# ELEKTRONN/ELEKTRONN2

Measured on AMD Instinct MI355X. Metric: training_input_voxels_per_sec, higher is better.
Workload: dtype f32; 1 GPU; neuro3d_lite (1,1,23,183,183)->(1,2,10,37,37) fwd+bwd+Adam, 1 sample/GPU; parallelism=dp1, hipgraph=True, steps_per_launch=10

## Files before the change

### elektronn2_amd/autotune.py

```python
from __future__ import annotations

import json
import math
import os

from .backend import E2Error

_HERE = os.path.dirname(os.path.abspath(__file__))
_SHIPPED = os.path.join(_HERE, "tuned.json")
_cache = None
_dirty = False
IGEMM_MTS = [1, 2, 3, 4, 5, 6, 7, 8, 10, 13]
WGRAD_MTS = [1, 2, 3, 4, 5, 7]


def _cache_path():
    return os.environ.get("E2HIP_TUNE_CACHE", os.path.join(_HERE, ".tune_cache.json"))


def _load():
    global _cache
    if _cache is None:
        _cache = {}
        for path in (_SHIPPED, _cache_path()):
# ... 101 lines not shown


def g4_pairs(mg, nt, kw):
    na = (4 * mg + 63) // 64
    u = 1
    while u < 8 and u * kw * mg * nt < 40 and 2 * (2 * u) * kw * (na + nt) + 4 * mg * nt <= 88:
        u *= 2
    return u


def igemm4_candidates(cout, cin, k, out_sp, split_k=True, n_cu=256):
    if k[2] not in (1, 3, 4, 5):
        return []
    q = out_sp[1] * out_sp[2]
    cinp = -(-cin // 4) * 4
    groups = -(-cout // 4)
    shapes = []
    for mg, nt in IGEMM4_INSTANCES:
        for wm in range(1, 13):
            bm = 4 * mg * wm
            nmt = -(-cout // bm)
            pad = nmt * bm - cout
            if pad >= 4 * mg and wm > 1:
                continue
            if nmt > 1 and wm < 3 and mg * wm < groups / 4.0:
                continue
            for wn in (1, 2, 3, 4, 6, 12):
                if wm * wn > 12 or (wm * wn < 6 and wm * wn != 4):
                    continue
                shapes.append((round(pad / float(cout), 3), -wm * wn, mg, nt, wm, wn, nmt))
    shapes.sort()
    best_pad = shapes[0][0] if shapes else 0
    cands = []
    for padf, _, mg, nt, wm, wn, nmt in shapes:
        if padf > best_pad + 0.06:
            break
        u = g4_pairs(mg, nt, k[2])
        step = u * 4 // math.gcd(u, 4)
        if ((step // u) * k[1]) % 2:
            step *= 2
        bn = 64 * nt * wn
        if bn > 2 * q:
            continue
        base = out_sp[0] * (-(-q // bn)) * nmt
        sks = (1,) if (base >= 160 or not split_k) else (1, 2, 4)
        ccs = sorted(set(-(-c // step) * step for c in (8, 16) if c >= 4))
        ccs = [c for c in ccs if -(-cin // c) * c <= cinp + 32][:2]
        for cc in ccs:
            for sk in sks:
                tiles = base * sk
                for g in (1, 2):
                    if g > 1 and (tiles <= n_cu or wm * wn > 6):
                        continue
                    cands.append("4,%d,%d,%d,%d,%d,%d,%d" % (mg, nt, cc, sk, wm, wn, g))
    return cands


def wgrad_candidates(cout, cin, k, out_sp, n_cu=256):
    mblocks = -(-cout // 16)
    T = k[0] * k[1] * k[2]
    nblocks = -(-(cin * T) // 16)
    q = out_sp[1] * out_sp[2]
    qpad = out_sp[1] * (out_sp[2] + 2 * (k[2] - 1))
    cands = []
    for mt in _best_mts(mblocks, WGRAD_MTS, keep=3):
        nmt = -(-mblocks // mt)
        variants = [(1, 1), (2, 1), (4, 1), (2, 14), (4, 14), (1, 0), (2, 0), (4, 0)]
        if nblocks <= 2:
            variants = [(1, 4), (1, 0), (1, 1), (2, 14)]
        for nt, wk in variants:
            wn = 1 if wk in (4, 14) else 4
            if nt > 1 and 16 * nt * wn > 16 * nblocks:
                continue
            nnt = -(-nblocks // (nt * wn))
            for bp in ((128, 256) if wk in (1, 14) else (64, 128)):
                tiles = out_sp[0] * (-(-(qpad if wk in (1, 14) else q) // bp))
                for fill in (1, 1.5, 2, 3, 4):
                    ps = max(1, min(tiles, int(n_cu * fill) // max(1, nmt * nnt)))
                    for q in {ps} | set(_near_divisors(tiles, ps)):
                        cands.append("%d,%d,%d,%d,%d" % (mt, nt, wk, bp, q))
                        if wk in (1, 14) and nnt >= 2 and nmt * q * nnt > 8:
                            cands.append("%d,%d,%d,%d,%d" % (mt, nt, wk + 100, bp, q))
    return sorted(set(cands) | set(pointwise_wgrad_candidates(cout, cin, k, out_sp, n_cu))
                  | set(position_split_wgrad_candidates(cout, cin, k, out_sp, n_cu)))


WGRAD_KS_TILES = [(13, 2), (10, 2), (8, 2), (8, 4), (7, 2), (7, 4), (6, 4), (5, 4), (4, 4), (3, 4), (2, 4)]


def position_split_wgrad_candidates(cout, cin, k, out_sp, n_cu=256):
    T = k[0] * k[1] * k[2]
    if T == 1 or cout < 24:
        return []
    pitch = out_sp[2] + k[2] - 1
    if (k[1] - 1) * pitch + k[2] - 1 < 31:
        return []
    units = out_sp[0] * (-(-((out_sp[1] - 1) * pitch + out_sp[2]) // 32))
    scored = []
    for mt, nt in WGRAD_KS_TILES:
        nm, nn = -(-cout // (16 * mt)), -(-(cin * T) // (16 * nt))
        eff = (cout * cin * T) / float(nm * 16 * mt * nn * 16 * nt)
        scored.append((-eff, -mt * nt, mt, nt, nm * nn))
    scored.sort()
    out = []
    for _, _, mt, nt, tiles in scored[:4]:
        for fill in (0.5, 1, 2):
            s = max(1, min(-(-units // 4), int(n_cu * fill) // tiles))
            out.append("%d,%d,9,0,%d" % (mt, nt, s))
    return sorted(set(out))


PW_WGRAD_KS_TILES = [(13, 2), (10, 2), (7, 2), (7, 4), (4, 4)]
PW_WGRAD_TILES = [(2, 2), (4, 2), (2, 4), (4, 4), (4, 3), (3, 4), (7, 2), (2, 7), (7, 4), (4, 7)]


def pointwise_wgrad_candidates(cout, cin, k, out_sp, n_cu=256):
    if tuple(k) != (1, 1, 1) or cout < 32 or cin < 32:
        return []
    steps = -(-(out_sp[0] * out_sp[1] * out_sp[2]) // 16)
    scored = []
    for mt, nt in PW_WGRAD_TILES:
        nm, nn = -(-cout // (32 * mt)), -(-cin // (32 * nt))
        eff = (cout * cin) / float(nm * 32 * mt * nn * 32 * nt)
        scored.append((-eff, mt * nt, mt, nt, nm * nn))
    scored.sort()
    out = []
    for _, _, mt, nt, tiles in scored[:5]:
        for fill in (0.5, 1, 2, 4):
            s = max(1, min(steps, int(n_cu * fill) // tiles))
            out.append("%d,%d,7,0,%d" % (mt, nt, s))
    units = max(1, (out_sp[0] * out_sp[1] * out_sp[2]) // 32)
    scored = []
    for mt, nt in PW_WGRAD_KS_TILES:
        nm, nn = -(-cout // (16 * mt)), -(-cin // (16 * nt))
        eff = (cout * cin) / float(nm * 16 * mt * nn * 16 * nt)
        scored.append((-eff, -mt * nt, mt, nt, nm * nn))
    scored.sort()
    for _, _, mt, nt, tiles in scored[:3]:
        for fill in (0.5, 0.75, 1, 2):
            s = max(1, min(-(-units // 4), int(n_cu * fill) // tiles))
            out.append("%d,%d,8,0,%d" % (mt, nt, s))
    return sorted(set(out))


_forced = {}
last_ranking = {}


def force(kind, cfg):
    if cfg:
        _forced[kind] = cfg
    else:
        _forced.pop(kind, None)


def known(ctx, kind, sig):
    if kind in _forced:
        return _forced[kind]
    suffix = "_bf16" if getattr(ctx, "mfma_dtype", "f32") == "bf16" else ""
    key = "%s%s|%s" % (kind, suffix, ",".join(str(int(v)) for v in sig))
    return _load().get(key)


def side_flag(ctx, sig):
    if getattr(ctx, "mfma_dtype", "f32") == "bf16":
        return False
    return _load().get("side|" + ",".join(str(int(v)) for v in sig)) == "1"


def set_side_flag(sig, on):
    global _dirty
    key = "side|" + ",".join(str(int(v)) for v in sig)
    c = _load()
    if on:
        c[key] = "1"
    else:
        c.pop(key, None)
    _dirty = True


def _time(ctx, fn, iters=4):
    fn()
    e0, e1 = ctx.event(), ctx.event()
    ctx.record(e0)
    for _ in range(iters):
        fn()
    ctx.record(e1)
    return ctx.elapsed_ms(e0, e1) / iters


fallbacks = []
# ... 89 lines not shown
```

### elektronn2_amd/csrc/common.hpp

```cpp
#pragma once
#include <hip/hip_runtime.h>
#include <stdint.h>
#include <stdio.h>
#include <stdlib.h>
#include <string>
#include "../../include/e2hip.h"

struct e2_ctx {
  int device;
  hipStream_t stream;
  int num_cu;
  bool capturing;
  float* zeros;
  hipEvent_t fork_ev[32];
  int fork_next;
  int mfma_bf16;
  int skip_zero_fill;
  float* last_fill_ptr;
  size_t last_fill_n;
  char tiling[2][64];
  int loss_sum_mode;
  float* loss_count_out;
  int input_slack;
  int image_rows;
// ... 44 lines not shown
  long esN, esD, esH;
};
#ifdef __HIPCC__
__device__ __forceinline__ float e2_uniform_ld(const float* p, int i) {
  return ((const __attribute__((address_space(4))) float*)p)[i];
}
#endif

static inline int e2i_nll_weights(const e2_nll_weights* w, const e2_tensor5* target,
                                  const char* who, NllW* out) {
  *out = NllW{};
  if (!w) return 0;
  out->cw = w->class_w; out->lab = w->labelled; out->npr = w->not_present;
  if (const e2_tensor5* e = w->example_w) {
    E2_REQUIRE(e->ptr && e->c == 1 && e->n == target->n && e->d == target->d &&
                   e->h == target->h && e->w == target->w,
               "%s: example_w must be (n,1,d,h,w) matching the target", who);
    out->ew = e->ptr; out->esN = e->sn; out->esD = e->sd; out->esH = e->sh;
  }
  return 0;
}

static inline int e2_cdiv(int a, int b) { return (a + b - 1) / b; }
static inline int64_t e2_cdiv64(int64_t a, int64_t b) { return (a + b - 1) / b; }


struct IgemmArgs {
  const float* in;
  const float* wp;
  float* out;
  int N, Cin, Cout;
  int kd, kh, kw;
  int Do, Ho, Wo;
  int64_t isN, isC, isZ, isY;
  int64_t osN, osC, osZ, osY;
  int ciP, coP;
  int upz, upy, upx;
  const float* bias = nullptr;
  int act = 0;
  const float* up_bias = nullptr;
  int up_act = 0;
  int* up_bias_done = nullptr;
  int gm = 0;
  const float* gm_src = nullptr;
  int64_t gsN = 0, gsC = 0, gsZ = 0;
  float* gm_dbias = nullptr;
  const float* gm_bias = nullptr;
  int* gm_done = nullptr;
  float* fill_base = nullptr;
  size_t fill_n = 0;
  int zpad = 0;
  int parts_max = 0;
  int64_t part_stride = 0;
  int* nparts = nullptr;
};
int e2i_igemm_conv(e2_ctx*, const IgemmArgs& a);
int e2i_pw_conv(e2_ctx*, const IgemmArgs& a, int MT, int NT, int KC);

int e2i_pack_weights(e2_ctx*, const float* w, float* wp, int Cout, int Cin,
                     int kd, int kh, int kw, int64_t wsO, int64_t wsI, int flip,
                     int ciP, int coP, int Rout, int Rin);
void e2i_pack_dims(int cout, int cin, int* ciP, int* coP);

struct WgradArgs {
  const float* x;
  const float* dy;
  float* dw;
  int N, Cin, Cout;
  int kd, kh, kw;
  int Do, Ho, Wo;
  int64_t xsN, xsC, xsZ, xsY;
  int64_t dsN, dsC, dsZ, dsY;
  int flip;
  int upR;
  int accumulate;
  int dy_padded;
};
int e2i_upconv_dpre_s2d(e2_ctx*, const e2_tensor5* dout, const e2_tensor5* yout, int pz,
                        int py, int px, int act, float* s2d, float* dbias);
int e2i_wgrad_conv(e2_ctx*, const WgradArgs& a);
int e2i_wgrad_direct(e2_ctx*, const WgradArgs& a, int MT, int NT, int BP, int PS, int WK, int xcd = 0);
int e2i_wgrad_direct_lpad(const WgradArgs& a, int BP);
int e2i_pw_wgrad(e2_ctx*, const WgradArgs& a, int MT, int NT, int S);
int e2i_pw_wgrad_ks(e2_ctx*, const WgradArgs& a, int MT, int NT, int S);
int e2i_wgrad_ks(e2_ctx*, const WgradArgs& a, int MT, int NT, int S);
size_t e2i_wgrad_direct_buf_floats(const WgradArgs& a, int NT, int BP, int WK);

int e2i_fill_view(e2_ctx*, const e2_tensor5* v, float value);
int e2i_fill_flat(e2_ctx*, float* ptr, size_t n, float value);
```

### elektronn2_amd/csrc/conv_pw_wgrad.hip

```cpp
#include "common.hpp"
#include <algorithm>
#include <type_traits>
#include <vector>
#include <cstdio>

typedef float f32x4 __attribute__((ext_vector_type(4)));

#ifdef E2_DEBUG_ENV
#define KS_STAMP(i) do { if (p.stamps && threadIdx.x == 0) p.stamps[8L * blockIdx.x + (i)] = __builtin_amdgcn_s_memtime(); } while (0)
#else
#define KS_STAMP(i) do {} while (0)
#endif

namespace {

struct PgP {
  const float* a; const float* b; float* c;
  long asN, asC, bsN, bsC;
  int N, M, Ncol, K;
  int R;
  int nMT, nNT, S;
  int stepsPerSample, steps, per;
  int rem;
  int T, kh, kw, flip, planes;
  long asZ, bsZ, bsY;
  unsigned long long* stamps;
};

__device__ __forceinline__ f32x4 pg_load(const float* row, int k, int K) {
  if (k + 3 < K) {
    f32x4 v;
    __builtin_memcpy(&v, row + k, 16);
    return v;
  }
  f32x4 v = {0.f, 0.f, 0.f, 0.f};
#pragma unroll
  for (int j = 0; j < 4; ++j)
    if (k + j < K) v[j] = row[k + j];
  return v;
}

template <int MT, int NT>
__global__ __launch_bounds__(256) void pw_wgrad_kernel(PgP p) {
  const int tid = threadIdx.x, lane = tid & 63, l15 = lane & 15, q = lane >> 4;
  const int wave = __builtin_amdgcn_readfirstlane(tid >> 6);
  const int wm = wave >> 1, wn = wave & 1;
  int b = blockIdx.x;
  const int nt = b % p.nNT; b /= p.nNT;
  const int mt = b % p.nMT;
  const int sp = b / p.nMT;
  const int m0 = (mt * 2 + wm) * 16 * MT;
  const int n0 = (nt * 2 + wn) * 16 * NT;
  const int s0 = sp * p.per, s1 = min(s0 + p.per, p.steps);

  long aoff[MT], boff[NT];
#pragma unroll
  for (int mb = 0; mb < MT; ++mb) aoff[mb] = (long)min(m0 + 16 * mb + l15, p.M - 1) * p.asC;
#pragma unroll
  for (int nb = 0; nb < NT; ++nb) boff[nb] = (long)min(n0 + 16 * nb + l15, p.Ncol - 1) * p.bsC;

  f32x4 acc[MT][NT];
#pragma unroll
  for (int mb = 0; mb < MT; ++mb)
#pragma unroll
    for (int nb = 0; nb < NT; ++nb) acc[mb][nb] = f32x4{0.f, 0.f, 0.f, 0.f};

  auto load = [&](int s, f32x4 (&A)[MT], f32x4 (&B)[NT]) {
    const int sc = min(s, s1 - 1);
    const int n = sc / p.stepsPerSample;
    const int k = (sc - n * p.stepsPerSample) * 16 + 4 * q;
    const float* ap = p.a + (long)n * p.asN;
    const float* bp = p.b + (long)n * p.bsN;
#pragma unroll
    for (int mb = 0; mb < MT; ++mb) A[mb] = pg_load(ap + aoff[mb], k, p.K);
#pragma unroll
    for (int nb = 0; nb < NT; ++nb) B[nb] = pg_load(bp + boff[nb], k, p.K);
  };
  auto fma = [&](const f32x4 (&A)[MT], const f32x4 (&B)[NT]) {
#pragma unroll
    for (int j = 0; j < 4; ++j)
#pragma unroll
      for (int mb = 0; mb < MT; ++mb)
#pragma unroll
// ... 125 lines not shown
    for (int mb = 0; mb < MT; ++mb) load2(A[mb], ap, aoff[mb] + kb);
    KS_STAMP(1);
#pragma unroll 1
    for (int i = 0; i < cnt; ++i) {
      where(min(i + 1, cnt - 1), ap, bp, kb, zb);
#pragma unroll
      for (int nb = 0; nb < NT; ++nb) load2(Bn[nb], bp, bo(nb, kb, zb));
#pragma unroll
      for (int mb = 0; mb < MT; ++mb) {
#pragma unroll
        for (int h = 0; h < 2; ++h)
#pragma unroll
          for (int j = 0; j < 4; ++j)
#pragma unroll
            for (int nb = 0; nb < NT; ++nb)
              acc[mb][nb] = __builtin_amdgcn_mfma_f32_16x16x4f32(A[mb][h][j], Bc[nb][h][j], acc[mb][nb], 0, 0, 0);
        load2(A[mb], ap, aoff[mb] + kb);
        __builtin_amdgcn_sched_barrier(0);
      }
#pragma unroll
      for (int nb = 0; nb < NT; ++nb) { Bc[nb][0] = Bn[nb][0]; Bc[nb][1] = Bn[nb][1]; }
#ifdef E2_DEBUG_ENV
      if (i == 0) KS_STAMP(2);
#endif
    }
  }
  KS_STAMP(3);
  if (!TAPS && sp == p.S - 1 && p.rem > 0) {
    constexpr int MBW = (MT + 3) / 4;
    const int k = p.K - p.rem + 4 * q;
#pragma unroll 1
    for (int n = 0; n < p.N; ++n) {
      float av[MBW][8], bv[NT][8];
      auto mload = [&](float (&d)[8], const float* row) {
#pragma unroll
        for (int e = 0; e < 8; ++e) {
          const int pos = k + (e >> 2) * 16 + (e & 3);
          const float v = row[min(pos, p.K - 1)];
          d[e] = pos < p.K ? v : 0.f;
        }
      };
#pragma unroll
      for (int nb = 0; nb < NT; ++nb)
        mload(bv[nb], p.b + (long)n * p.bsN + (long)min(n0 + 16 * nb + l15, p.Ncol - 1) * p.bsC);
#pragma unroll
      for (int i = 0; i < MBW; ++i)
        mload(av[i], p.a + (long)n * p.asN + (long)min(m0 + 16 * min(wave + 4 * i, MT - 1) + l15, p.M - 1) * p.asC);
#pragma unroll
      for (int mb = 0; mb < MT; ++mb)
        if ((mb & 3) == wave) {
#pragma unroll
          for (int e = 0; e < 8; ++e)
#pragma unroll
            for (int nb = 0; nb < NT; ++nb)
              acc[mb][nb] = __builtin_amdgcn_mfma_f32_16x16x4f32(av[mb >> 2][e], bv[nb][e], acc[mb][nb], 0, 0, 0);
        }
    }
  }

  float* mine = red + wave * RS;
#pragma unroll
  for (int mb = 0; mb < MT; ++mb)
#pragma unroll
    for (int nb = 0; nb < NT; ++nb)
#pragma unroll
      for (int r = 0; r < 4; ++r) mine[(16 * mb + 4 * q + r) * RW + 16 * nb + l15] = acc[mb][nb][r];
  __syncthreads();
  KS_STAMP(4);
#pragma unroll 2
  for (int e = tid; e < 16 * MT * 16 * NT; e += 256) {
    const int ml = e / (16 * NT), nl = e - ml * (16 * NT);
    const int m = m0 + ml, n = n0 + nl;
    const float* s = red + ml * RW + nl;
    const float v = (s[0] + s[RS]) + (s[2 * RS] + s[3 * RS]);
    if (m >= p.M || n >= p.Ncol) continue;
    float* dst = dst_of(m, n);
    if (single) *dst += v;
    else unsafeAtomicAdd(dst, v);
  }
  KS_STAMP(5);
#ifdef E2_DEBUG_ENV
  if (p.stamps) { __builtin_amdgcn_s_waitcnt(0); KS_STAMP(6); }
#endif
}

template <int MT, int NT, bool TAPS = false>
int launch_ks(e2_ctx* ctx, const PgP& p, long grid) {
  const int lds = 4 * 16 * MT * (16 * NT + 4) * (int)sizeof(float);
  static bool raised = false;
  if (!raised) {
    hipError_t e = hipFuncSetAttribute(reinterpret_cast<const void*>(&pw_wgrad_ks_kernel<MT, NT, TAPS>),
                                       hipFuncAttributeMaxDynamicSharedMemorySize, lds);
    if (e != hipSuccess) { e2_set_error("hipFuncSetAttribute: %s", hipGetErrorString(e)); return 1; }
    raised = true;
  }
#ifdef E2_DEBUG_ENV
  PgP ps = p;
  const bool stamps = e2_dbg_env("E2_PWKS_STAMPS") != nullptr && !ctx->capturing;
  if (stamps) {
    E2_CHECK_HIP(hipMalloc(&ps.stamps, sizeof(unsigned long long) * 8 * grid));
    E2_CHECK_HIP(hipMemsetAsync(ps.stamps, 0, sizeof(unsigned long long) * 8 * grid, ctx->stream));
  }
  hipLaunchKernelGGL((pw_wgrad_ks_kernel<MT, NT, TAPS>), dim3((unsigned)grid), dim3(256), lds, ctx->stream, ps);
  E2_CHECK_HIP(hipGetLastError());
  if (stamps) {
    E2_CHECK_HIP(hipStreamSynchronize(ctx->stream));
    std::vector<unsigned long long> h(8 * grid);
    E2_CHECK_HIP(hipMemcpy(h.data(), ps.stamps, sizeof(unsigned long long) * 8 * grid, hipMemcpyDeviceToHost));
    static const char* names[6] = {"prologue issue", "first unit", "other units", "LDS + barrier", "flush issue", "flush done"};
    double sum[6] = {0};
    unsigned long long t0 = ~0ull, t1 = 0, s1 = 0;
    long nb = 0;
    for (long b = 0; b < grid; ++b) {
      if (!h[8 * b + 6]) continue;
      ++nb;
      for (int i = 0; i < 6; ++i) sum[i] += (double)(h[8 * b + i + 1] - h[8 * b + i]);
      t0 = std::min(t0, h[8 * b]); t1 = std::max(t1, h[8 * b + 6]); s1 = std::max(s1, h[8 * b]);
    }
    fprintf(stderr, "[e2] pw_wgrad_ks<%d,%d> grid %ld (%ld main), S %d, per %d: first start -> last end %llu ticks, last start %llu\n",
            MT, NT, grid, nb, p.S, p.per, t1 - t0, s1 - t0);
    for (int i = 0; i < 6; ++i) fprintf(stderr, "   %-14s %9.0f ticks\n", names[i], sum[i] / std::max(1L, nb));
    (void)hipFree(ps.stamps);
  }
#else
  hipLaunchKernelGGL((pw_wgrad_ks_kernel<MT, NT, TAPS>), dim3((unsigned)grid), dim3(256), lds, ctx->stream, p);
  E2_CHECK_HIP(hipGetLastError());
#endif
  return 0;
}

template <int MT, int NT>
int launch(e2_ctx* ctx, const PgP& p, long grid) {
  hipLaunchKernelGGL((pw_wgrad_kernel<MT, NT>), dim3((unsigned)grid), dim3(256), 0, ctx->stream, p);
  E2_CHECK_HIP(hipGetLastError());
  return 0;
}

}

int e2i_pw_wgrad(e2_ctx* ctx, const WgradArgs& a, int MT, int NT, int S) {
  E2_REQUIRE(a.kd == 1 && a.kh == 1 && a.kw == 1, "pointwise wgrad: kernel %dx%dx%d is not 1x1x1", a.kd, a.kh, a.kw);
  E2_REQUIRE(a.xsY == a.Wo && a.xsZ == (int64_t)a.Ho * a.Wo && a.dsY == a.Wo && a.dsZ == (int64_t)a.Ho * a.Wo,
             "pointwise wgrad: x and dy need dense channel planes (row stride = W, plane stride = H * W)");
  E2_REQUIRE(!ctx->mfma_bf16, "pointwise wgrad: an f32 kernel, not offered in bf16 mode");
  PgP p;
  p.a = a.dy; p.b = a.x; p.c = a.dw;
  p.asN = a.dsN; p.asC = a.dsC; p.bsN = a.xsN; p.bsC = a.xsC;
  p.N = a.N; p.M = a.Cout; p.Ncol = a.Cin;
  const long K = (long)a.Do * a.Ho * a.Wo;
  E2_REQUIRE(K < (1L << 30), "pointwise wgrad: sample too large");
  p.K = (int)K;
  p.R = a.upR > 1 ? a.upR : 1;
  E2_REQUIRE(a.Cout % p.R == 0, "pointwise wgrad: %d rows for %d sub-positions", a.Cout, p.R);
  p.nMT = e2_cdiv(a.Cout, 32 * MT);
  p.nNT = e2_cdiv(a.Cin, 32 * NT);
  p.rem = 0; p.stamps = nullptr;
  p.T = 1; p.kh = p.kw = 1; p.flip = 0; p.planes = 1; p.asZ = p.bsZ = p.bsY = 0;
  p.stepsPerSample = (int)((K + 15) / 16);
  const long steps = (long)a.N * p.stepsPerSample;
  E2_REQUIRE(steps < (1L << 30), "pointwise wgrad: too many positions");
  p.steps = (int)steps;
  S = (int)std::max<long>(1, std::min<long>(S, steps));
  p.per = (int)((steps + S - 1) / S);
  p.S = (int)((steps + p.per - 1) / p.per);
  const long grid = (long)p.nMT * p.nNT * p.S;
  E2_REQUIRE(grid < (1L << 31), "pointwise wgrad: grid too large");
  if (!a.accumulate)
    if (int rc = e2i_fill_flat(ctx, a.dw, (size_t)a.Cout * a.Cin, 0.f)) return rc;
#define E2_L(M, N_) if (MT == M && NT == N_) return launch<M, N_>(ctx, p, grid);
  E2_L(2, 2) E2_L(4, 2) E2_L(2, 4) E2_L(4, 4) E2_L(4, 3) E2_L(3, 4) E2_L(7, 2) E2_L(2, 7) E2_L(7, 4) E2_L(4, 7)
#undef E2_L
  e2_set_error("pointwise wgrad: no instance MT=%d NT=%d", MT, NT);
  return 2;
}

int e2i_pw_wgrad_ks(e2_ctx* ctx, const WgradArgs& a, int MT, int NT, int S) {
  E2_REQUIRE(a.kd == 1 && a.kh == 1 && a.kw == 1, "pointwise wgrad: kernel %dx%dx%d is not 1x1x1", a.kd, a.kh, a.kw);
  E2_REQUIRE(a.xsY == a.Wo && a.xsZ == (int64_t)a.Ho * a.Wo && a.dsY == a.Wo && a.dsZ == (int64_t)a.Ho * a.Wo,
             "pointwise wgrad: x and dy need dense channel planes (row stride = W, plane stride = H * W)");
  E2_REQUIRE(!ctx->mfma_bf16, "pointwise wgrad: an f32 kernel, not offered in bf16 mode");
  PgP p;
  p.a = a.dy; p.b = a.x; p.c = a.dw;
  p.asN = a.dsN; p.asC = a.dsC; p.bsN = a.xsN; p.bsC = a.xsC;
  p.N = a.N; p.M = a.Cout; p.Ncol = a.Cin;
  const long K = (long)a.Do * a.Ho * a.Wo;
  E2_REQUIRE(K >= 4 && K < (1L << 30), "pointwise wgrad: sample of %ld positions", K);
  E2_REQUIRE(((long)a.Cout * a.dsC + K) * 4 < (1L << 32) && ((long)a.Cin * a.xsC + K) * 4 < (1L << 32) && a.dsC >= 0 && a.xsC >= 0,
             "pointwise wgrad: sample too large for 32-bit byte offsets");
  p.K = (int)K;
  p.R = a.upR > 1 ? a.upR : 1;
  E2_REQUIRE(a.Cout % p.R == 0, "pointwise wgrad: %d rows for %d sub-positions", a.Cout, p.R);
  p.nMT = e2_cdiv(a.Cout, 16 * MT);
  p.nNT = e2_cdiv(a.Cin, 16 * NT);
  p.stepsPerSample = (int)(K / 32);
  p.rem = (int)(K % 32); p.stamps = nullptr;
  p.T = 1; p.kh = p.kw = 1; p.flip = 0; p.planes = 1; p.asZ = p.bsZ = p.bsY = 0;
  const long units = (long)a.N * p.stepsPerSample;
  E2_REQUIRE(units < (1L << 29), "pointwise wgrad: too many positions");
  p.steps = (int)units;
  S = (int)std::max<long>(1, std::min<long>(S, std::max<long>(1, (units + 3) / 4)));
  p.per = (int)std::max<long>(1, (units + S - 1) / S);
  p.per = (p.per + 3) & ~3;
  p.S = (int)std::max<long>(1, (units + p.per - 1) / p.per);
  long grid = (long)p.nMT * p.nNT * p.S;
  grid = (grid + 7) & ~7L;
  E2_REQUIRE(grid < (1L << 31), "pointwise wgrad: grid too large");
  if (!a.accumulate)
    if (int rc = e2i_fill_flat(ctx, a.dw, (size_t)a.Cout * a.Cin, 0.f)) return rc;
#define E2_L(M, N_) if (MT == M && NT == N_) return launch_ks<M, N_>(ctx, p, grid);
  E2_L(13, 2) E2_L(7, 2) E2_L(7, 4) E2_L(4, 4) E2_L(10, 2)
#undef E2_L
  e2_set_error("pointwise wgrad (position-split waves): no instance MT=%d NT=%d", MT, NT);
  return 2;
}

int e2i_wgrad_ks(e2_ctx* ctx, const WgradArgs& a, int MT, int NT, int S) {
  const int T = a.kd * a.kh * a.kw;
  E2_REQUIRE(T > 1 && a.upR <= 1, "wgrad (position-split GEMM): a conv kernel with taps");
  E2_REQUIRE(a.dy_padded, "wgrad (position-split GEMM): dy must be the interior of its zero-padded buffer");
  E2_REQUIRE(a.dsY == a.xsY, "wgrad (position-split GEMM): dy rows at the input's pitch (%ld vs %ld)", (long)a.dsY, (long)a.xsY);
  E2_REQUIRE((a.kh - 1) * a.xsY + (a.kw - 1) >= 31, "wgrad (position-split GEMM): %d x %d kernel rows of %ld leave fewer than 31 zeros behind a plane",
             a.kh, a.kw, (long)a.xsY);
  E2_REQUIRE(!ctx->mfma_bf16, "wgrad (position-split GEMM): an f32 kernel, not offered in bf16 mode");
  const int Din = a.Do + a.kd - 1, Hin = a.Ho + a.kh - 1;
  E2_REQUIRE(a.xsZ >= (int64_t)Hin * a.xsY && a.xsC >= (int64_t)Din * a.xsZ, "wgrad (position-split GEMM): x planes / channels overlap");
  PgP p;
  p.a = a.dy; p.b = a.x; p.c = a.dw;
  p.asN = a.dsN; p.asC = a.dsC; p.bsN = a.xsN; p.bsC = a.xsC;
  p.N = a.N; p.M = a.Cout; p.Ncol = a.Cin * T;
  const long K = (long)(a.Ho - 1) * a.dsY + a.Wo;
  E2_REQUIRE(K >= 4 && K < (1L << 28), "wgrad (position-split GEMM): plane of %ld positions", K);
  E2_REQUIRE(((long)a.Cout * a.dsC + (long)a.Do * a.dsZ + K) * 4 + 256 < (1L << 32) &&
                 ((long)a.Cin * a.xsC + (long)Din * a.xsZ) * 4 + 256 < (1L << 32) && a.dsC >= 0 && a.xsC >= 0,
             "wgrad (position-split GEMM): sample too large for 32-bit byte offsets");
  p.K = (int)K; p.R = 1; p.rem = 0; p.stamps = nullptr;
  p.T = T; p.kh = a.kh; p.kw = a.kw; p.flip = a.flip; p.planes = a.Do;
  p.asZ = a.dsZ; p.bsZ = a.xsZ; p.bsY = a.xsY;
  E2_REQUIRE(ctx->input_slack >= 128, "wgrad (position-split GEMM): needs e2_set_input_slack(ctx, >= 128)");
#ifdef E2_DEBUG_ENV
  if (!ctx->capturing) {
    const float* end = a.x + (int64_t)(a.N - 1) * a.xsN + (int64_t)(a.Cin - 1) * a.xsC +
                       (int64_t)(Din - 1) * a.xsZ + (int64_t)(Hin - 1) * a.xsY + (a.Wo + a.kw - 1);
    float h[32];
    E2_CHECK_HIP(hipStreamSynchronize(ctx->stream));
    E2_CHECK_HIP(hipMemcpy(h, end, sizeof(h), hipMemcpyDeviceToHost));
    for (int i = 0; i < 32; ++i)
      E2_REQUIRE(h[i] == h[i] && h[i] - h[i] == 0.f, "wgrad (position-split GEMM): e2_set_input_slack promised finite "
                 "values behind x, but float %d behind its last element is %g", i, (double)h[i]);
  }
#endif
  p.nMT = e2_cdiv(a.Cout, 16 * MT);
  p.nNT = e2_cdiv(p.Ncol, 16 * NT);
  p.stepsPerSample = (int)((K + 31) / 32);
  const long units = (long)a.N * a.Do * p.stepsPerSample;
  E2_REQUIRE(units < (1L << 29), "wgrad (position-split GEMM): too many positions");
  p.steps = (int)units;
  S = (int)std::max<long>(1, std::min<long>(S, std::max<long>(1, (units + 3) / 4)));
  p.per = (int)std::max<long>(1, (units + S - 1) / S);
  p.per = (p.per + 3) & ~3;
  p.S = (int)std::max<long>(1, (units + p.per - 1) / p.per);
  long grid = (long)p.nMT * p.nNT * p.S;
  grid = (grid + 7) & ~7L;
  E2_REQUIRE(grid < (1L << 31), "wgrad (position-split GEMM): grid too large");
  if (!a.accumulate)
    if (int rc = e2i_fill_flat(ctx, a.dw, (size_t)a.Cout * p.Ncol, 0.f)) return rc;
#define E2_L(M, N_) if (MT == M && NT == N_) return launch_ks<M, N_, true>(ctx, p, grid);
  E2_L(13, 2) E2_L(7, 2) E2_L(7, 4) E2_L(4, 4) E2_L(10, 2) E2_L(5, 4) E2_L(3, 4) E2_L(2, 4) E2_L(8, 2) E2_L(8, 4) E2_L(6, 4)
#undef E2_L
  e2_set_error("wgrad (position-split GEMM): no instance MT=%d NT=%d", MT, NT);
  return 2;
}
```

### elektronn2_amd/csrc/conv_wgrad.hip

```cpp
#include "stream_common.hpp"
#include <stdlib.h>
#include <algorithm>
#include <utility>

typedef float f32x4 __attribute__((ext_vector_type(4)));
typedef int i32x4 __attribute__((ext_vector_type(4)));
typedef __attribute__((address_space(3))) void* lds_vp;
typedef const __attribute__((address_space(1))) void* gbl_vp;

__device__ __forceinline__ void w_glds4(const float* g, float* l) {
  __builtin_amdgcn_global_load_lds((gbl_vp)g, (lds_vp)l, 4, 0, 0);
}
__device__ __forceinline__ void w_glds16(const float* g, float* l) {
  __builtin_amdgcn_global_load_lds((gbl_vp)g, (lds_vp)l, 16, 0, 0);
}
template <int OFF>
__device__ __forceinline__ float w_lds_ld(unsigned addr) {
  float v;
  asm volatile("ds_read_b32 %0, %1 offset:%2" : "=v"(v) : "v"(addr), "i"(OFF));
  return v;
}
__device__ __forceinline__ i32x4 w_lds_ld128(unsigned addr) {
  i32x4 v;
  asm volatile("ds_read_b128 %0, %1" : "=v"(v) : "v"(addr));
// ... 388 lines not shown
          const int nPT = (int)((S + BP - 1) / BP);
          const long tiles = (long)a.N * a.Do * nPT;
          const long base = (long)nMT * nNT;
          for (int fill = 1; fill <= 2; ++fill) {
            long PS = std::max<long>(1, ((long)slots * fill + base - 1) / base);
            PS = std::min(PS, tiles);
            const int per = (int)((tiles + PS - 1) / PS);
            const double tile = (BP / 4.0) * MT * NT * 35.0 + (BP / 16.0) * 150.0 + 1200.0;
            const double flush = 16.0 * MT * 16.0 * NT * 4 * 0.6;
            const double wg_time = per * tile + flush + 5000.0;
            const long wgs = base * PS;
            const double rounds = (double)((wgs + slots - 1) / slots);
            const double atom = (double)PS * dw_bytes / 1.3e12 * 2.4e9 + dw_bytes / 4e12 * 2.4e9;
            const double cost = rounds * wg_time + atom;
            if (cost < bestCost) { bestCost = cost; best = WCfg{MT, NT, 1, BP, (int)PS}; }
          }
        }
      }
    }
    if (best.MT) { *ok = 1; return best; }
  }
  for (int MT : kWMTs) {
    if (MT > mblocks && MT != 1) continue;
    const int nMT = e2_cdiv(mblocks, MT);
    for (int v = 0; v < 4; ++v) {
      const int NT = (v == 3) ? 1 : (1 << v);
      const int WK = (v == 3) ? 4 : 1;
      const int WN = 4 / WK;
      const int BNn = 16 * NT * WN;
      if (16 * NT * WN > 16 * nblocks && NT > 1) continue;
      if (WK == 4 && nblocks > 2) continue;
      const int nNT = e2_cdiv(nblocks, NT * WN);
      for (int BP = 64; BP <= 128; BP *= 2) {
        if (BP == 128 && Q <= 64) continue;
        const size_t bufF = w_buf_floats(a, MT, BNn, BP);
        const size_t lds = 2 * bufF * 4;
        if (lds > 160 * 1024) continue;
        const int perCU = lds <= 80 * 1024 ? 2 : 1;
        const int slots = ctx->num_cu * perCU;
        const int nPT = (int)((Q + BP - 1) / BP);
        const long tiles = (long)a.N * a.Do * nPT;
        const long base = (long)nMT * nNT;
        for (int fill = 1; fill <= 2; ++fill) {
          long PS = std::max<long>(1, ((long)slots * fill + base - 1) / base);
          PS = std::min(PS, tiles);
          const int per = (int)((tiles + PS - 1) / PS);
          const double mfma = (BP / 4.0 / WK) * MT * NT * 32.0;
          const double bytes = 4.0 * (16.0 * MT * BP + (double)w_maxspans(a, BNn) * w_lmax(a, BP));
          const double issue = (BP / 4.0 / WK) * (MT + 2.0 * NT + 1) * 5.0;
          double tile = std::max(mfma, issue) * perCU * 1.08 + 400.0;
          tile = std::max(tile, bytes / 20.0 * perCU);
          const double flush = 16.0 * MT * 16.0 * NT * 4 * WK * 0.6;
          const double wg_time = per * tile + flush + 5000.0;
          const long wgs = base * PS;
          const double rounds = (double)((wgs + slots - 1) / slots);
          const double atom = (double)PS * dw_bytes * WK / 1.3e12 * 2.4e9 + dw_bytes / 4e12 * 2.4e9;
          const double cost = rounds * wg_time + atom;
          if (cost < bestCost) { bestCost = cost; best = WCfg{MT, NT, WK, BP, (int)PS}; }
        }
      }
    }
  }
  *ok = best.MT != 0;
  return best;
}

int e2i_wgrad_conv(e2_ctx* ctx, const WgradArgs& a) {
  E2_REQUIRE(a.Do > 0 && a.Ho > 0 && a.Wo > 0 && a.Cin > 0 && a.Cout > 0,
             "wgrad: empty problem");
  E2_REQUIRE(a.xsY < (1 << 20), "wgrad: input row stride too large");
  int ok = 0, src = E2_SRC_MODEL;
  WCfg c = choose_wcfg(ctx, a, &ok, &src);
  E2_REQUIRE(ok, "wgrad: no tiling fits LDS (Cin=%d Cout=%d k=%dx%dx%d)", a.Cin, a.Cout,
             a.kd, a.kh, a.kw);
  {
    const bool direct = a.dy_padded && (c.WK == 1 || c.WK == 14 || c.WK == 101 || c.WK == 114) &&
                        (c.BP == 128 || c.BP == 256);
    const char* fam = c.WK == 7 ? "pw_wgrad" : c.WK == 8 ? "pw_wgrad_ks" : c.WK == 9 ? "wgrad_ks"
                      : direct ? (ctx->mfma_bf16 ? "wgrad_direct_bf16r" : "wgrad_direct")
                      : "wgrad_lds";
    e2_note_launch(ctx, fam, src, "%d,%d,%d,%d,%d", c.MT, c.NT, c.WK, c.BP, c.PS);
  }
  if (c.WK == 7) return e2i_pw_wgrad(ctx, a, c.MT, c.NT, c.PS);
  if (c.WK == 8) return e2i_pw_wgrad_ks(ctx, a, c.MT, c.NT, c.PS);
  if (c.WK == 9) return e2i_wgrad_ks(ctx, a, c.MT, c.NT, c.PS);
  if (a.dy_padded && (c.WK == 1 || c.WK == 14 || c.WK == 101 || c.WK == 114) && (c.BP == 128 || c.BP == 256))
    return e2i_wgrad_direct(ctx, a, c.MT, c.NT, c.BP, c.PS, (c.WK % 100) == 14 ? 4 : 1, c.WK >= 100);
  E2_REQUIRE(c.WK != 14 && c.WK < 100, "wgrad: WK=14/101/114 need the padded-gradient entry point and BP 128/256");
  if (c.WK == 0) c.WK = 1;
  E2_REQUIRE(c.BP == 64 || c.BP == 128, "wgrad: BP must be 64 or 128");
  E2_REQUIRE(c.WK == 1 || (c.WK == 4 && c.NT == 1), "wgrad: WK=4 needs NT=1");
  WgradP p;
  p.x = a.x; p.dy = a.dy; p.dw = a.dw;
  p.zeros = ctx->zeros;
  p.Cin = a.Cin; p.Cout = a.Cout; p.kd = a.kd; p.kh = a.kh; p.kw = a.kw;
  p.THW = a.kh * a.kw; p.T = a.kd * p.THW;
  p.Do = a.Do; p.Ho = a.Ho; p.Wo = a.Wo; p.Q = a.Ho * a.Wo;
  p.xsN = a.xsN; p.xsC = a.xsC; p.xsZ = a.xsZ; p.xsY = a.xsY;
  p.dsN = a.dsN; p.dsC = a.dsC; p.dsZ = a.dsZ; p.dsY = a.dsY;
  p.flip = a.flip;
  p.upR = a.upR > 1 ? a.upR : 1;
  const long NTOT = (long)a.Cin * p.T;
  E2_REQUIRE(NTOT < (1L << 30), "wgrad: Cin*T too large");
  p.NTOT = (int)NTOT;
  const int WN = 4 / c.WK;
  const int BNn = 16 * c.NT * WN;
  p.Lpad = w_lpad(w_lmax(a, c.BP));
  p.maxSpans = w_maxspans(a, BNn);
  p.nMT = e2_cdiv(e2_cdiv(a.Cout, 16), c.MT);
  p.nNT = e2_cdiv(e2_cdiv(p.NTOT, 16), c.NT * WN);
  p.nPT = e2_cdiv(p.Q, c.BP);
  p.tilesTotal = a.N * a.Do * p.nPT;
  p.nPS = std::max(1, std::min(c.PS, p.tilesTotal));
  p.bufFloats = (int)w_buf_floats(a, c.MT, BNn, c.BP);
  p.Din = a.Do + a.kd - 1;
  p.N = a.N;
  p.divWo = mk_div((unsigned)a.Wo);
  p.dbg = e2_dbg_env_int("E2_WGRAD_DBG");
  p.bf16 = (ctx->mfma_bf16 && a.dy_padded) ? 1 : 0;
  size_t lds = 2 * (size_t)p.bufFloats * 4;
  lds += (size_t)e2_dbg_env_int("E2_WGRAD_LDSPAD");
  E2_REQUIRE(lds <= 160 * 1024, "wgrad: tiling needs %zu B of LDS", lds);
  const long grid = (long)p.nMT * p.nNT * p.nPS;
  E2_REQUIRE(grid < (1L << 31), "wgrad: grid too large");
  if (!a.accumulate)
    if (int rc = e2i_fill_flat(ctx, a.dw, (size_t)a.Cout * p.NTOT, 0.f)) return rc;
  if (e2_dbg_env("E2_VERBOSE"))
    fprintf(stderr, "[e2] wgrad%s Cin=%d Cout=%d k=%d,%d,%d out=%d,%d,%d MT=%d NT=%d WK=%d BP=%d PS=%d grid=%ld lds=%zu\n",
            p.bf16 ? "(bf16)" : "", a.Cin, a.Cout, a.kd, a.kh, a.kw, a.Do, a.Ho, a.Wo, c.MT, c.NT, c.WK, c.BP, p.nPS, grid, lds);
  return dispatch_w(ctx, p, c.MT, c.NT, c.BP, c.WK, (int)grid, lds);
}
```

Before: 520.9 million voxels/s.

## Add even-split work distribution for position-split wgrad kernels

Adds a new wgrad kernel variant that splits the (tile, position-unit) pair space evenly across a fixed number of work-groups, so each group walks contiguous segments across tile boundaries and atomically accumulates partial results. The aim is to remove load imbalance and tail effects of the existing per-tile position split. New autotune candidates encode the band count in the BP field. The default path only changes if the tuner picks these candidates, and the variant adds extra atomics and an LDS reduction per segment.

```diff
diff --git a/elektronn2_amd/autotune.py b/elektronn2_amd/autotune.py
--- a/elektronn2_amd/autotune.py
+++ b/elektronn2_amd/autotune.py
@@ -207,7 +207,8 @@
                         if wk in (1, 14) and nnt >= 2 and nmt * q * nnt > 8:
                             cands.append("%d,%d,%d,%d,%d" % (mt, nt, wk + 100, bp, q))
     return sorted(set(cands) | set(pointwise_wgrad_candidates(cout, cin, k, out_sp, n_cu))
-                  | set(position_split_wgrad_candidates(cout, cin, k, out_sp, n_cu)))
+                  | set(position_split_wgrad_candidates(cout, cin, k, out_sp, n_cu))
+                  | set(even_split_wgrad_candidates(cout, cin, k, out_sp, n_cu)))
 
 
 WGRAD_KS_TILES = [(13, 2), (10, 2), (8, 2), (8, 4), (7, 2), (7, 4), (6, 4), (5, 4), (4, 4), (3, 4), (2, 4)]
@@ -232,6 +233,35 @@
         for fill in (0.5, 1, 2):
             s = max(1, min(-(-units // 4), int(n_cu * fill) // tiles))
             out.append("%d,%d,9,0,%d" % (mt, nt, s))
+    return sorted(set(out))
+
+
+def even_split_wgrad_candidates(cout, cin, k, out_sp, n_cu=256):
+    T = k[0] * k[1] * k[2]
+    if T == 1:
+        if cout < 32 or cin < 32 or out_sp[0] * out_sp[1] * out_sp[2] < 32:
+            return []
+        tiles, form = PW_WGRAD_KS_TILES, 8
+        units = out_sp[0] * out_sp[1] * out_sp[2] // 32
+    else:
+        if not position_split_wgrad_candidates(cout, cin, k, out_sp, n_cu):
+            return []
+        tiles, form = WGRAD_KS_TILES, 9
+        pitch = out_sp[2] + k[2] - 1
+        units = out_sp[0] * (-(-((out_sp[1] - 1) * pitch + out_sp[2]) // 32))
+    scored = []
+    for mt, nt in tiles:
+        nm, nn = -(-cout // (16 * mt)), -(-(cin * T) // (16 * nt))
+        eff = (cout * cin * T) / float(nm * 16 * mt * nn * 16 * nt)
+        scored.append((-eff, -mt * nt, mt, nt, nm * nn))
+    scored.sort()
+    out = []
+    for _, _, mt, nt, ntiles in scored[:3]:
+        lds = 4 * 16 * mt * (16 * nt + 4) * 4
+        for r in range(1, min(2, (160 * 1024) // lds) + 1):
+            g = n_cu * r
+            for b in sorted({1, max(1, min(-(-units // 4), g // ntiles))}):
+                out.append("%d,%d,%d,%d,%d" % (mt, nt, form, b, g))
     return sorted(set(out))
 
 
diff --git a/elektronn2_amd/csrc/common.hpp b/elektronn2_amd/csrc/common.hpp
--- a/elektronn2_amd/csrc/common.hpp
+++ b/elektronn2_amd/csrc/common.hpp
@@ -150,8 +150,8 @@
 int e2i_wgrad_direct(e2_ctx*, const WgradArgs& a, int MT, int NT, int BP, int PS, int WK, int xcd = 0);
 int e2i_wgrad_direct_lpad(const WgradArgs& a, int BP);
 int e2i_pw_wgrad(e2_ctx*, const WgradArgs& a, int MT, int NT, int S);
-int e2i_pw_wgrad_ks(e2_ctx*, const WgradArgs& a, int MT, int NT, int S);
-int e2i_wgrad_ks(e2_ctx*, const WgradArgs& a, int MT, int NT, int S);
+int e2i_pw_wgrad_ks(e2_ctx*, const WgradArgs& a, int MT, int NT, int S, int even);
+int e2i_wgrad_ks(e2_ctx*, const WgradArgs& a, int MT, int NT, int S, int even);
 size_t e2i_wgrad_direct_buf_floats(const WgradArgs& a, int NT, int BP, int WK);
 
 int e2i_fill_view(e2_ctx*, const e2_tensor5* v, float value);
diff --git a/elektronn2_amd/csrc/conv_pw_wgrad.hip b/elektronn2_amd/csrc/conv_pw_wgrad.hip
--- a/elektronn2_amd/csrc/conv_pw_wgrad.hip
+++ b/elektronn2_amd/csrc/conv_pw_wgrad.hip
@@ -1,4 +1,5 @@
 #include "common.hpp"
+#include "wgrad_even.hpp"
 #include <algorithm>
 #include <type_traits>
 #include <vector>
@@ -290,6 +291,231 @@
 #ifdef E2_DEBUG_ENV
   if (p.stamps) { __builtin_amdgcn_s_waitcnt(0); KS_STAMP(6); }
 #endif
+}
+
+template <int MT, int NT, bool TAPS>
+__global__ __launch_bounds__(256) void pw_wgrad_ev_kernel(PgP p, WgEven ev) {
+  extern __shared__ float red[];
+  constexpr int RW = 16 * NT + 4;
+  constexpr int RS = 16 * MT * RW;
+  const int tid = threadIdx.x, lane = tid & 63, l15 = lane & 15, q = lane >> 4;
+  const int wave = __builtin_amdgcn_readfirstlane(tid >> 6);
+  int g = blockIdx.x;
+  if ((ev.G & 7) == 0) g = (g & 7) * (ev.G >> 3) + (g >> 3);
+  WgRange rg = wg_even_range(ev, g);
+  if (rg.b >= rg.e) return;
+  KS_STAMP(0);
+#ifdef E2_DEBUG_ENV
+  int nseg = 0;
+#endif
+#pragma unroll 1
+  do {
+    const WgSeg sg = wg_even_seg(ev, rg);
+    const int mt = sg.tile / p.nNT, nt = sg.tile - mt * p.nNT;
+    const int m0 = mt * 16 * MT, n0 = nt * 16 * NT;
+    const int u0 = sg.u0 + wave, u1 = sg.u0 + sg.n;
+    const int cnt = u0 < u1 ? (u1 - u0 + 3) >> 2 : 0;
+
+    unsigned aoff[MT], boff[NT];
+#pragma unroll
+    for (int mb = 0; mb < MT; ++mb) aoff[mb] = (unsigned)min(m0 + 16 * mb + l15, p.M - 1) * (unsigned)p.asC * 4u + 16u * q;
+#pragma unroll
+    for (int nb = 0; nb < NT; ++nb) {
+      const int j = min(n0 + 16 * nb + l15, p.Ncol - 1);
+      if (TAPS) {
+        const int ci = j / p.T, ts = j - ci * p.T;
+        const int t = p.flip ? p.T - 1 - ts : ts;
+        const int tz = t / (p.kh * p.kw), r2 = t - tz * (p.kh * p.kw);
+        const int ty = r2 / p.kw, tx = r2 - ty * p.kw;
+        const unsigned row = (unsigned)ci * (unsigned)p.bsC * 4u;
+        boff[nb] = row + (unsigned)(tz * p.bsZ + ty * p.bsY + tx) * 4u + 16u * q;
+      } else {
+        boff[nb] = (unsigned)j * (unsigned)p.bsC * 4u + 16u * q;
+      }
+    }
+
+    f32x4 acc[MT][NT];
+#pragma unroll
+    for (int mb = 0; mb < MT; ++mb)
+#pragma unroll
+      for (int nb = 0; nb < NT; ++nb) acc[mb][nb] = f32x4{0.f, 0.f, 0.f, 0.f};
+
+    auto where = [&](int i, const char*& ap, const char*& bp, unsigned& kb, unsigned& zb) {
+      const int u = u0 + 4 * i;
+      const int pl = u / p.stepsPerSample;
+      kb = (unsigned)(u - pl * p.stepsPerSample) * 128u;
+      if (TAPS) {
+        const int n = pl / p.planes, z = pl - n * p.planes;
+        ap = reinterpret_cast<const char*>(p.a + (long)n * p.asN + (long)z * p.asZ);
+        bp = reinterpret_cast<const char*>(p.b + (long)n * p.bsN);
+        zb = (unsigned)(z * p.bsZ) * 4u;
+      } else {
+        ap = reinterpret_cast<const char*>(p.a + (long)pl * p.asN);
+        bp = reinterpret_cast<const char*>(p.b + (long)pl * p.bsN);
+        zb = 0;
+      }
+    };
+    auto bo = [&](int nb, unsigned kb, unsigned zb) -> unsigned {
+      return TAPS ? boff[nb] + zb + kb : boff[nb] + kb;
+    };
+    auto load2 = [&](f32x4 (&d)[2], const char* base, unsigned off) {
+      const char* r = base + off;
+      __builtin_memcpy(&d[0], r, 16);
+      __builtin_memcpy(&d[1], r + 64, 16);
+    };
+
+    if (cnt > 0) {
+      f32x4 A[MT][2], Bc[NT][2], Bn[NT][2];
+      const char *ap, *bp;
+      unsigned kb, zb;
+      where(0, ap, bp, kb, zb);
+#pragma unroll
+      for (int nb = 0; nb < NT; ++nb) load2(Bc[nb], bp, bo(nb, kb, zb));
+#pragma unroll
+      for (int mb = 0; mb < MT; ++mb) load2(A[mb], ap, aoff[mb] + kb);
+#pragma unroll 1
+      for (int i = 0; i < cnt; ++i) {
+        where(min(i + 1, cnt - 1), ap, bp, kb, zb);
+#pragma unroll
+        for (int nb = 0; nb < NT; ++nb) load2(Bn[nb], bp, bo(nb, kb, zb));
+#pragma unroll
+        for (int mb = 0; mb < MT; ++mb) {
+#pragma unroll
+          for (int h = 0; h < 2; ++h)
+#pragma unroll
+            for (int j = 0; j < 4; ++j)
+#pragma unroll
+              for (int nb = 0; nb < NT; ++nb)
+                acc[mb][nb] = __builtin_amdgcn_mfma_f32_16x16x4f32(A[mb][h][j], Bc[nb][h][j], acc[mb][nb], 0, 0, 0);
+          load2(A[mb], ap, aoff[mb] + kb);
+          __builtin_amdgcn_sched_barrier(0);
+        }
+#pragma unroll
+        for (int nb = 0; nb < NT; ++nb) { Bc[nb][0] = Bn[nb][0]; Bc[nb][1] = Bn[nb][1]; }
+      }
+    }
+    if (!TAPS && u1 == ev.U && p.rem > 0) {
+      constexpr int MBW = (MT + 3) / 4;
+      const int k = p.K - p.rem + 4 * q;
+#pragma unroll 1
+      for (int n = 0; n < p.N; ++n) {
+        float av[MBW][8], bv[NT][8];
+        auto mload = [&](float (&d)[8], const float* row) {
+#pragma unroll
+          for (int e = 0; e < 8; ++e) {
+            const int pos = k + (e >> 2) * 16 + (e & 3);
+            const float v = row[min(pos, p.K - 1)];
+            d[e] = pos < p.K ? v : 0.f;
+          }
+        };
+#pragma unroll
+        for (int nb = 0; nb < NT; ++nb)
+          mload(bv[nb], p.b + (long)n * p.bsN + (long)min(n0 + 16 * nb + l15, p.Ncol - 1) * p.bsC);
+#pragma unroll
+        for (int i = 0; i < MBW; ++i)
+          mload(av[i], p.a + (long)n * p.asN + (long)min(m0 + 16 * min(wave + 4 * i, MT - 1) + l15, p.M - 1) * p.asC);
+#pragma unroll
+        for (int mb = 0; mb < MT; ++mb)
+          if ((mb & 3) == wave) {
+#pragma unroll
+            for (int e = 0; e < 8; ++e)
+#pragma unroll
+              for (int nb = 0; nb < NT; ++nb)
+                acc[mb][nb] = __builtin_amdgcn_mfma_f32_16x16x4f32(av[mb >> 2][e], bv[nb][e], acc[mb][nb], 0, 0, 0);
+          }
+      }
+    }
+
+    float* mine = red + wave * RS;
+#pragma unroll
+    for (int mb = 0; mb < MT; ++mb)
+#pragma unroll
+      for (int nb = 0; nb < NT; ++nb)
+#pragma unroll
+        for (int r = 0; r < 4; ++r) mine[(16 * mb + 4 * q + r) * RW + 16 * nb + l15] = acc[mb][nb][r];
+    __syncthreads();
+#pragma unroll 2
+    for (int e = tid; e < 16 * MT * 16 * NT; e += 256) {
+      const int ml = e / (16 * NT), nl = e - ml * (16 * NT);
+      const int m = m0 + ml, n = n0 + nl;
+      const float* s = red + ml * RW + nl;
+      const float v = (s[0] + s[RS]) + (s[2 * RS] + s[3 * RS]);
+      if (m >= p.M || n >= p.Ncol) continue;
+      float* dst;
+      if (p.R > 1) { const int co = m / p.R; dst = p.c + (long)co * p.Ncol * p.R + (m - co * p.R) + (long)n * p.R; }
+      else dst = p.c + (long)m * p.Ncol + n;
+      unsafeAtomicAdd(dst, v);
+    }
+    __syncthreads();
+#ifdef E2_DEBUG_ENV
+    ++nseg;
+#endif
+    rg.b += sg.n;
+  } while (rg.b < rg.e);
+#ifdef E2_DEBUG_ENV
+  if (p.stamps) {
+    __builtin_amdgcn_s_waitcnt(0);
+    KS_STAMP(6);
+    if (threadIdx.x == 0) p.stamps[8L * blockIdx.x + 7] = (unsigned long long)nseg;
+  }
+#endif
+}
+
+template <int MT, int NT, bool TAPS>
+int launch_ev(e2_ctx* ctx, const PgP& p, const WgEven& ev) {
+  const int lds = 4 * 16 * MT * (16 * NT + 4) * (int)sizeof(float);
+  static bool raised = false;
+  if (!raised) {
+    hipError_t e = hipFuncSetAttribute(reinterpret_cast<const void*>(&pw_wgrad_ev_kernel<MT, NT, TAPS>),
+                                       hipFuncAttributeMaxDynamicSharedMemorySize, lds);
+    if (e != hipSuccess) { e2_set_error("hipFuncSetAttribute: %s", hipGetErrorString(e)); return 1; }
+    raised = true;
+  }
+  PgP ps = p;
+#ifdef E2_DEBUG_ENV
+  const long grid = ev.G;
+  const bool stamps = e2_dbg_env("E2_PWKS_STAMPS") != nullptr && !ctx->capturing;
+  if (stamps) {
+    E2_CHECK_HIP(hipMalloc(&ps.stamps, sizeof(unsigned long long) * 8 * grid));
+    E2_CHECK_HIP(hipMemsetAsync(ps.stamps, 0, sizeof(unsigned long long) * 8 * grid, ctx->stream));
+  }
+#endif
+  hipLaunchKernelGGL((pw_wgrad_ev_kernel<MT, NT, TAPS>), dim3((unsigned)ev.G), dim3(256), lds, ctx->stream, ps, ev);
+  E2_CHECK_HIP(hipGetLastError());
+#ifdef E2_DEBUG_ENV
+  if (stamps) {
+    E2_CHECK_HIP(hipStreamSynchronize(ctx->stream));
+    std::vector<unsigned long long> h(8 * grid);
+    E2_CHECK_HIP(hipMemcpy(h.data(), ps.stamps, sizeof(unsigned long long) * 8 * grid, hipMemcpyDeviceToHost));
+    unsigned long long t0 = ~0ull, t1 = 0;
+    double sum[2] = {0, 0}, mx[2] = {0, 0};
+    long cntw[2] = {0, 0};
+    for (long b = 0; b < grid; ++b) {
+      if (!h[8 * b + 6]) continue;
+      const int k = h[8 * b + 7] > 1;
+      const double d = (double)(h[8 * b + 6] - h[8 * b]);
+      sum[k] += d; mx[k] = std::max(mx[k], d); ++cntw[k];
+      t0 = std::min(t0, h[8 * b]); t1 = std::max(t1, h[8 * b + 6]);
+    }
+    fprintf(stderr, "[e2] pw_wgrad_ev<%d,%d> G %d, %d tiles x %d units in %d bands, %d(+1 for %d) pairs each: first start -> last end %llu ticks\n",
+            MT, NT, ev.G, ev.T, ev.U, ev.B, ev.base, ev.extra, t1 - t0);
+    for (int k = 0; k < 2; ++k)
+      fprintf(stderr, "   %-22s %5ld work-groups, mean %9.0f max %9.0f ticks\n", k ? "two or more segments" : "one segment",
+              cntw[k], sum[k] / std::max(1L, cntw[k]), mx[k]);
+    (void)hipFree(ps.stamps);
+  }
+#endif
+  return 0;
+}
+
+static int even_split(const PgP& p, long G, int B, WgEven* ev) {
+  const long T = (long)p.nMT * p.nNT;
+  E2_REQUIRE(p.steps >= 1, "wgrad (even position ranges): no whole 32-position unit");
+  E2_REQUIRE(T * p.steps < (1L << 31), "wgrad (even position ranges): too many (tile, unit) pairs");
+  E2_REQUIRE(G >= 1 && G <= (1L << 16), "wgrad (even position ranges): %ld work-groups (1 .. 65536)", G);
+  E2_REQUIRE(B >= 1 && B <= p.steps, "wgrad (even position ranges): %d bands for %d units", B, p.steps);
+  *ev = wg_even_make((int)T, p.steps, (int)G, B);
+  return 0;
 }
 
 template <int MT, int NT, bool TAPS = false>
@@ -382,7 +608,7 @@
   return 2;
 }
 
-int e2i_pw_wgrad_ks(e2_ctx* ctx, const WgradArgs& a, int MT, int NT, int S) {
+int e2i_pw_wgrad_ks(e2_ctx* ctx, const WgradArgs& a, int MT, int NT, int S, int even) {
   E2_REQUIRE(a.kd == 1 && a.kh == 1 && a.kw == 1, "pointwise wgrad: kernel %dx%dx%d is not 1x1x1", a.kd, a.kh, a.kw);
   E2_REQUIRE(a.xsY == a.Wo && a.xsZ == (int64_t)a.Ho * a.Wo && a.dsY == a.Wo && a.dsZ == (int64_t)a.Ho * a.Wo,
              "pointwise wgrad: x and dy need dense channel planes (row stride = W, plane stride = H * W)");
@@ -406,6 +632,7 @@
   const long units = (long)a.N * p.stepsPerSample;
   E2_REQUIRE(units < (1L << 29), "pointwise wgrad: too many positions");
   p.steps = (int)units;
+  const long S0 = S;
   S = (int)std::max<long>(1, std::min<long>(S, std::max<long>(1, (units + 3) / 4)));
   p.per = (int)std::max<long>(1, (units + S - 1) / S);
   p.per = (p.per + 3) & ~3;
@@ -413,16 +640,19 @@
   long grid = (long)p.nMT * p.nNT * p.S;
   grid = (grid + 7) & ~7L;
   E2_REQUIRE(grid < (1L << 31), "pointwise wgrad: grid too large");
+  WgEven ev{};
+  if (even > 0)
+    if (int rc = even_split(p, S0, even, &ev)) return rc;
   if (!a.accumulate)
     if (int rc = e2i_fill_flat(ctx, a.dw, (size_t)a.Cout * a.Cin, 0.f)) return rc;
-#define E2_L(M, N_) if (MT == M && NT == N_) return launch_ks<M, N_>(ctx, p, grid);
+#define E2_L(M, N_) if (MT == M && NT == N_) return even > 0 ? launch_ev<M, N_, false>(ctx, p, ev) : launch_ks<M, N_>(ctx, p, grid);
   E2_L(13, 2) E2_L(7, 2) E2_L(7, 4) E2_L(4, 4) E2_L(10, 2)
 #undef E2_L
   e2_set_error("pointwise wgrad (position-split waves): no instance MT=%d NT=%d", MT, NT);
   return 2;
 }
 
-int e2i_wgrad_ks(e2_ctx* ctx, const WgradArgs& a, int MT, int NT, int S) {
+int e2i_wgrad_ks(e2_ctx* ctx, const WgradArgs& a, int MT, int NT, int S, int even) {
   const int T = a.kd * a.kh * a.kw;
   E2_REQUIRE(T > 1 && a.upR <= 1, "wgrad (position-split GEMM): a conv kernel with taps");
   E2_REQUIRE(a.dy_padded, "wgrad (position-split GEMM): dy must be the interior of its zero-padded buffer");
@@ -463,6 +693,7 @@
   const long units = (long)a.N * a.Do * p.stepsPerSample;
   E2_REQUIRE(units < (1L << 29), "wgrad (position-split GEMM): too many positions");
   p.steps = (int)units;
+  const long S0 = S;
   S = (int)std::max<long>(1, std::min<long>(S, std::max<long>(1, (units + 3) / 4)));
   p.per = (int)std::max<long>(1, (units + S - 1) / S);
   p.per = (p.per + 3) & ~3;
@@ -470,9 +701,12 @@
   long grid = (long)p.nMT * p.nNT * p.S;
   grid = (grid + 7) & ~7L;
   E2_REQUIRE(grid < (1L << 31), "wgrad (position-split GEMM): grid too large");
+  WgEven ev{};
+  if (even > 0)
+    if (int rc = even_split(p, S0, even, &ev)) return rc;
   if (!a.accumulate)
     if (int rc = e2i_fill_flat(ctx, a.dw, (size_t)a.Cout * p.Ncol, 0.f)) return rc;
-#define E2_L(M, N_) if (MT == M && NT == N_) return launch_ks<M, N_, true>(ctx, p, grid);
+#define E2_L(M, N_) if (MT == M && NT == N_) return even > 0 ? launch_ev<M, N_, true>(ctx, p, ev) : launch_ks<M, N_, true>(ctx, p, grid);
   E2_L(13, 2) E2_L(7, 2) E2_L(7, 4) E2_L(4, 4) E2_L(10, 2) E2_L(5, 4) E2_L(3, 4) E2_L(2, 4) E2_L(8, 2) E2_L(8, 4) E2_L(6, 4)
 #undef E2_L
   e2_set_error("wgrad (position-split GEMM): no instance MT=%d NT=%d", MT, NT);
diff --git a/elektronn2_amd/csrc/conv_wgrad.hip b/elektronn2_amd/csrc/conv_wgrad.hip
--- a/elektronn2_amd/csrc/conv_wgrad.hip
+++ b/elektronn2_amd/csrc/conv_wgrad.hip
@@ -494,8 +494,8 @@
     e2_note_launch(ctx, fam, src, "%d,%d,%d,%d,%d", c.MT, c.NT, c.WK, c.BP, c.PS);
   }
   if (c.WK == 7) return e2i_pw_wgrad(ctx, a, c.MT, c.NT, c.PS);
-  if (c.WK == 8) return e2i_pw_wgrad_ks(ctx, a, c.MT, c.NT, c.PS);
-  if (c.WK == 9) return e2i_wgrad_ks(ctx, a, c.MT, c.NT, c.PS);
+  if (c.WK == 8) return e2i_pw_wgrad_ks(ctx, a, c.MT, c.NT, c.PS, c.BP);
+  if (c.WK == 9) return e2i_wgrad_ks(ctx, a, c.MT, c.NT, c.PS, c.BP);
   if (a.dy_padded && (c.WK == 1 || c.WK == 14 || c.WK == 101 || c.WK == 114) && (c.BP == 128 || c.BP == 256))
     return e2i_wgrad_direct(ctx, a, c.MT, c.NT, c.BP, c.PS, (c.WK % 100) == 14 ? 4 : 1, c.WK >= 100);
   E2_REQUIRE(c.WK != 14 && c.WK < 100, "wgrad: WK=14/101/114 need the padded-gradient entry point and BP 128/256");
diff --git a/elektronn2_amd/csrc/wgrad_even.hpp b/elektronn2_amd/csrc/wgrad_even.hpp
--- /dev/null
+++ b/elektronn2_amd/csrc/wgrad_even.hpp
@@ -0,0 +1,37 @@
+#pragma once
+
+#if defined(__HIPCC__)
+#define E2_WG_HD __host__ __device__
+#else
+#define E2_WG_HD
+#endif
+
+struct WgEven {
+  int T, U, G;
+  int B, per;
+  int base, extra;
+};
+struct WgRange { int b, e; };
+struct WgSeg { int tile, u0, n; };
+
+E2_WG_HD inline WgEven wg_even_make(int T, int U, int G, int B) {
+  const long total = (long)T * U;
+  int per = (U + B - 1) / B;
+  per = (per + 3) & ~3;
+  return WgEven{T, U, G, (U + per - 1) / per, per, (int)(total / G), (int)(total % G)};
+}
+
+E2_WG_HD inline WgRange wg_even_range(const WgEven& ev, int g) {
+  const int b = g * ev.base + (g < ev.extra ? g : ev.extra);
+  return WgRange{b, b + ev.base + (g < ev.extra ? 1 : 0)};
+}
+
+E2_WG_HD inline WgSeg wg_even_seg(const WgEven& ev, const WgRange& r) {
+  const int full = (ev.B - 1) * ev.T * ev.per;
+  int band, i, len;
+  if (r.b < full) { band = r.b / (ev.T * ev.per); i = r.b - band * (ev.T * ev.per); len = ev.per; }
+  else { band = ev.B - 1; i = r.b - full; len = ev.U - band * ev.per; }
+  const int tile = i / len, off = i - tile * len;
+  const int left = r.e - r.b, room = len - off;
+  return WgSeg{tile, band * ev.per + off, left < room ? left : room};
+}
```

Result: faster. 527.6 million voxels/s (median of 6 runs) (+1.3%).
